# Deci-AI/super-gradients

Hardware: AMD Instinct MI355X
Metric: images/sec/node YOLO-NAS-S 640x640 train-step (higher is better)
Workload: dtype fp32 (bf16x3 MFMA); 1 GPU; YOLO-NAS-S synthetic COCO 640x640, bs=32/GPU, PPYoloELoss(TAL)+AdamW+EMA, random-init weights; global_batch=32, parallelism=dp1, conv_math=patch_bf3, conv_variant=0, bn_reduce_in_data_gradients=True, conv_tuning_entries=374, filter_planes=True

## Files before the change

### super_gradients_amd/csrc/bn.hip

```cpp
#include "sgx_common.h"
#include <atomic>

#include "sgx_sweep.h"

extern "C" int32_t sgx_stats_blocks(int64_t M) {
    long n = (M + 63) / 64;
    if (n < 1) n = 1;
    if (n > 1024) n = 1024;
    return (int32_t)n;
}

struct StatsF {
    const float* x;
    long ld;
    struct In { float4 v; };
    __device__ In load(long r, int c) const { return In{sgx_ld4(x + r * ld + c)}; }
    struct Cst {};
    __device__ Cst consts(int) const { return Cst{}; }
    __device__ void apply(long, int, const In& in, const Cst&, float4 (&q)[2]) const {
        const float4 v = in.v;
        q[0].x += v.x; q[0].y += v.y; q[0].z += v.z; q[0].w += v.w;
        q[1].x += v.x * v.x; q[1].y += v.y * v.y; q[1].z += v.z * v.z; q[1].w += v.w * v.w;
    }
};
// ... 821 lines not shown
                                          int32_t C, int32_t act, float* partials, int32_t nblk, void* stream) {
    SGX_CHECK_ARG(x1 && s1 && t1 && y, "tri_affine_act_fwd: null pointer");
    SGX_CHECK_ACT3(act, "tri_affine_act_fwd");
    SGX_CHECK_ARG(!x2 || (s2 && t2), "tri_affine_act_fwd: second branch needs scale and shift");
    SGX_CHECK_ARG(!x3 || (s3 && t3), "tri_affine_act_fwd: third branch needs scale and shift");
    SW_CHECK_VEC(C, SW_LD4(x1_ld) && (!x2 || SW_LD4(x2_ld)) && (!x3 || SW_LD4(x3_ld)) && (!r || SW_LD4(r_ld)) && SW_LD4(y_ld) && SW_ALIGNED(x1) && SW_ALIGNED(s1) && SW_ALIGNED(t1) &&
                     (!x2 || (SW_ALIGNED(x2) && SW_ALIGNED(s2) && SW_ALIGNED(t2))) && (!x3 || (SW_ALIGNED(x3) && SW_ALIGNED(s3) && SW_ALIGNED(t3))) && SW_ALIGNED(r) &&
                     SW_ALIGNED(y) && SW_ALIGNED(partials),
                 "tri_affine_act_fwd");
    Branch br[3] = {{x1, x1_ld, s1, t1, nullptr}, {x2, x2_ld, s2, t2, nullptr}, {x3, x3_ld, s3, t3, nullptr}};
    const int nb = present(br);
    const BranchSumOut o{r, r_ld, r_scale, r_scale_dev, y, y_ld};
    return nb == 1 ? branch_sum_fwd<1>(br, act, o, M, C, partials, nblk, stream)
         : nb == 2 ? branch_sum_fwd<2>(br, act, o, M, C, partials, nblk, stream)
                   : branch_sum_fwd<3>(br, act, o, M, C, partials, nblk, stream);
}

template <int NB>
struct BranchSumBwdReduceF {
    BranchSum<NB> p; const float* dy; long dy_ld; float* g; long g_ld;
    struct In { float4 x[NB], d; };
    struct Cst { typename BranchSum<NB>::Cst k; float4 m[NB]; };
    __device__ In load(long row, int c) const {
        In in;
        p.load(row, c, in.x);
        in.d = sgx_ld4(dy + row * dy_ld + c);
        return in;
    }
    __device__ Cst consts(int c) const {
        Cst k;
        k.k = p.consts(c);
#pragma unroll
        for (int i = 0; i < NB; ++i) k.m[i] = sgx_ld4(p.b[i].mean + c);
        return k;
    }
    __device__ float4 grad(const float4& d, const float4& v) const {
#pragma clang fp contract(off)
        return make_float4(d.x * sgx_act_grad(v.x, p.act), d.y * sgx_act_grad(v.y, p.act), d.z * sgx_act_grad(v.z, p.act), d.w * sgx_act_grad(v.w, p.act));
    }
    __device__ void apply(long row, int c, const In& in, const Cst& k, float4 (&q)[2 * NB]) const {
        const float4 o = grad(in.d, p.pre(k.k, in.x));
        sgx_st4(g + row * g_ld + c, o);
#pragma unroll
        for (int i = 0; i < NB; ++i) {
            const float4 e = in.x[i], m = k.m[i];
            q[2 * i].x += o.x; q[2 * i].y += o.y; q[2 * i].z += o.z; q[2 * i].w += o.w;
            q[2 * i + 1].x += o.x * (e.x - m.x); q[2 * i + 1].y += o.y * (e.y - m.y); q[2 * i + 1].z += o.z * (e.z - m.z); q[2 * i + 1].w += o.w * (e.w - m.w);
        }
    }
};
template <int NB>
static int32_t branch_sum_bwd_reduce(const Branch* br, int act, const float* dy, long dy_ld, float* g, long g_ld, long M, int C, float* partials,
                                     int nblk, void* stream) {
    return run_sweep<BranchSumBwdReduceF<NB>, 2 * NB, 2>({branch_sum<NB>(br, act), dy, dy_ld, g, g_ld}, M, C, partials, stream, "tri_affine_act_bwd_reduce", nblk);
}
extern "C" int32_t sgx_tri_affine_act_bwd_reduce(const float* dy, int64_t dy_ld, const float* x1, int64_t x1_ld, const float* s1, const float* t1,
                                                 const float* mean1, const float* x2, int64_t x2_ld, const float* s2, const float* t2,
                                                 const float* mean2, const float* x3, int64_t x3_ld, const float* s3, const float* t3,
                                                 const float* mean3, float* g, int64_t g_ld, int64_t M, int32_t C, int32_t act, float* partials,
                                                 int32_t nblk, void* stream) {
    SGX_CHECK_ARG(dy && x1 && s1 && t1 && mean1 && g && partials, "tri_affine_act_bwd_reduce: null pointer");
    SGX_CHECK_ACT3(act, "tri_affine_act_bwd_reduce");
    SGX_CHECK_ARG(!x2 || (s2 && t2 && mean2), "tri_affine_act_bwd_reduce: second branch needs scale, shift and mean");
    SGX_CHECK_ARG(!x3 || (s3 && t3 && mean3), "tri_affine_act_bwd_reduce: third branch needs scale, shift and mean");
    SW_CHECK_VEC(C, SW_LD4(dy_ld) && SW_LD4(x1_ld) && (!x2 || SW_LD4(x2_ld)) && (!x3 || SW_LD4(x3_ld)) && SW_LD4(g_ld) && SW_ALIGNED(dy) && SW_ALIGNED(x1) && SW_ALIGNED(s1) &&
                     SW_ALIGNED(t1) && SW_ALIGNED(mean1) && (!x2 || (SW_ALIGNED(x2) && SW_ALIGNED(s2) && SW_ALIGNED(t2) && SW_ALIGNED(mean2))) &&
                     (!x3 || (SW_ALIGNED(x3) && SW_ALIGNED(s3) && SW_ALIGNED(t3) && SW_ALIGNED(mean3))) && SW_ALIGNED(g) && SW_ALIGNED(partials),
                 "tri_affine_act_bwd_reduce");
    Branch br[3] = {{x1, x1_ld, s1, t1, mean1}, {x2, x2_ld, s2, t2, mean2}, {x3, x3_ld, s3, t3, mean3}};
    const int nb = present(br);
    return nb == 1 ? branch_sum_bwd_reduce<1>(br, act, dy, dy_ld, g, g_ld, M, C, partials, nblk, stream)
         : nb == 2 ? branch_sum_bwd_reduce<2>(br, act, dy, dy_ld, g, g_ld, M, C, partials, nblk, stream)
                   : branch_sum_bwd_reduce<3>(br, act, dy, dy_ld, g, g_ld, M, C, partials, nblk, stream);
}

struct ColsumF {
    const float* x; long ld; long rows_per_img; long ld_img;
    struct In { float4 v; };
    __device__ In load(long r, int c) const {
        long img = r / rows_per_img;
        return In{sgx_ld4(x + img * ld_img + (r - img * rows_per_img) * ld + c)};
    }
    struct Cst {};
    __device__ Cst consts(int) const { return Cst{}; }
    __device__ void apply(long, int, const In& in, const Cst&, float4 (&q)[1]) const {
        const float4 v = in.v;
        q[0].x += v.x; q[0].y += v.y; q[0].z += v.z; q[0].w += v.w;
    }
};
__global__ void colsum_finalize_kernel(ColSrc src, int C, float* out, int accumulate) {
    SGX_FIN_THREAD(src, C);
    double tot[1];
    col_totals<1>(src, C, c, cok, tot);
    if (!writer) return;
    const double s = tot[0];
    out[c] = accumulate ? out[c] + (float)s : (float)s;
}
extern "C" int64_t sgx_colsum_workspace(int64_t M, int32_t C) {
    int nblk = sgx_stats_blocks(M);
    return (((int64_t)nblk * C * (int64_t)sizeof(float) + 255) & ~255L) + sgx_reduce_workspace(nblk, C);
}
extern "C" int32_t sgx_colsum(const float* x, int64_t ld, int64_t M, int32_t C, int64_t rows_per_img, int64_t ld_img, float* out,
                              int32_t accumulate, float* ws, void* stream) {
    SGX_CHECK_ARG(x && out && ws && rows_per_img > 0, "colsum: bad args");
    SW_CHECK_VEC(C, SW_LD4(ld) && SW_LD4(ld_img) && SW_ALIGNED(x) && SW_ALIGNED(ws), "colsum");
    ColsumF f{x, ld, rows_per_img, ld_img};
    int32_t rc = run_sweep<ColsumF, 1, 4>(f, M, C, ws, stream, "colsum");
    if (rc) return rc;
    const int nblk = sgx_stats_blocks(M);
    const int64_t part_bytes = ((int64_t)nblk * C * (int64_t)sizeof(float) + 255) & ~255L;
    ColSrc src;
    rc = col_prereduce<1>(ws, nblk, C, (char*)ws + part_bytes, sgx_reduce_workspace(nblk, C), stream, &src);
    if (rc) return rc;
    SGX_LAUNCH(colsum_finalize_kernel, fin_grid(src, C), fin_block(src), 0, stream, src, C, out, accumulate);
    SGX_CHECK_LAUNCH("colsum_finalize");
    return SGX_OK;
}

__global__ void fill_kernel(float* p, long n, float v) {
    for (long i = (long)blockIdx.x * blockDim.x + threadIdx.x; i < n; i += (long)gridDim.x * blockDim.x) p[i] = v;
}
extern "C" int32_t sgx_fill(float* p, int64_t n, float v, void* stream) {
    if (n <= 0) return SGX_OK;
    SGX_CHECK_ARG(p, "fill: null pointer");
    long blocks = (n + 255) / 256;
    SGX_LAUNCH(fill_kernel, dim3((unsigned)(blocks > 4096 ? 4096 : blocks)), dim3(256), 0, stream, p, (long)n, v);
    SGX_CHECK_LAUNCH("fill");
    return SGX_OK;
}

__global__ void scale_dev_kernel(const float* x, const float* s, const float* t, float* y, long n) {
    float f = s[0] * (t ? t[0] : 1.f);
    for (long i = (long)blockIdx.x * blockDim.x + threadIdx.x; i < n; i += (long)gridDim.x * blockDim.x) y[i] = x[i] * f;
}
extern "C" int32_t sgx_scale_by_device_scalar(const float* x, const float* s, const float* t, float* y, int64_t n, void* stream) {
    if (n <= 0) return SGX_OK;
    SGX_CHECK_ARG(x && s && y, "scale: null pointer");
    long blocks = (n + 255) / 256;
    SGX_LAUNCH(scale_dev_kernel, dim3((unsigned)(blocks > 4096 ? 4096 : blocks)), dim3(256), 0, stream, x, s, t, y, (long)n);
    SGX_CHECK_LAUNCH("scale_by_device_scalar");
    return SGX_OK;
}

__global__ void nchw_to_nhwc_kernel(int N, int C, int H, int W, int Cpad, const float* x, float* y) {
    long n = (long)N * H * W * Cpad;
    for (long i = (long)blockIdx.x * blockDim.x + threadIdx.x; i < n; i += (long)gridDim.x * blockDim.x) {
        int c = (int)(i % Cpad);
        long pix = i / Cpad;
        long hw = (long)H * W;
        long img = pix / hw, rem = pix - img * hw;
        y[i] = c < C ? x[(img * C + c) * hw + rem] : 0.f;
    }
}
extern "C" int32_t sgx_nchw_to_nhwc(int32_t N, int32_t C, int32_t H, int32_t W, int32_t Cpad, const float* x, float* y, void* stream) {
    SGX_CHECK_ARG(x && y && Cpad >= C && Cpad % 4 == 0, "nchw_to_nhwc: bad args");
    long n = (long)N * H * W * Cpad, blocks = (n + 255) / 256;
    SGX_LAUNCH(nchw_to_nhwc_kernel, dim3((unsigned)(blocks > 8192 ? 8192 : blocks)), dim3(256), 0, stream, N, C, H, W, Cpad, x, y);
    SGX_CHECK_LAUNCH("nchw_to_nhwc");
    return SGX_OK;
}
__global__ void nhwc_to_nchw_kernel(int N, int C, int H, int W, const float* x, long ld_pix, long ld_img, float* y) {
    long n = (long)N * C * H * W;
    long hw = (long)H * W;
    for (long i = (long)blockIdx.x * blockDim.x + threadIdx.x; i < n; i += (long)gridDim.x * blockDim.x) {
        long rem = i % hw;
        long t = i / hw;
        int c = (int)(t % C);
        long img = t / C;
        y[i] = x[img * ld_img + rem * ld_pix + c];
    }
}
extern "C" int32_t sgx_nhwc_to_nchw(int32_t N, int32_t C, int32_t H, int32_t W, const float* x, int64_t x_ld_pix, int64_t x_ld_img, float* y,
                                    void* stream) {
    SGX_CHECK_ARG(x && y, "nhwc_to_nchw: null pointer");
    long n = (long)N * C * H * W, blocks = (n + 255) / 256;
    SGX_LAUNCH(nhwc_to_nchw_kernel, dim3((unsigned)(blocks > 8192 ? 8192 : blocks)), dim3(256), 0, stream, N, C, H, W, x, (long)x_ld_pix,
               (long)x_ld_img, y);
    SGX_CHECK_LAUNCH("nhwc_to_nchw");
    return SGX_OK;
}

__global__ void standardize_u8_kernel(long npix, int C, int Cpad, const uint8_t* x, float max_value, const float* mean, const float* stdv, float* y) {
    for (long i = (long)blockIdx.x * blockDim.x + threadIdx.x; i < npix; i += (long)gridDim.x * blockDim.x) {
        const uint8_t* px = x + i * C;
        float* py = y + i * Cpad;
        for (int c0 = 0; c0 < Cpad; c0 += 4) {
            float v[4];
#pragma unroll
            for (int t = 0; t < 4; ++t) {
                const int c = c0 + t;
                float f = 0.f;
                if (c < C) {
                    f = (float)px[c] / max_value;
                    if (mean) f = (f - mean[c]) / stdv[c];
                }
                v[t] = f;
            }
            sgx_st4(py + c0, make_float4(v[0], v[1], v[2], v[3]));
        }
    }
}
extern "C" int32_t sgx_standardize_u8_hwc(int32_t N, int32_t H, int32_t W, int32_t C, int32_t Cpad, const uint8_t* x, float max_value,
                                          const float* mean, const float* stdv, float* y, void* stream) {
    SGX_CHECK_ARG(x && y && N > 0 && H > 0 && W > 0 && C > 0 && Cpad >= C && Cpad % 4 == 0, "standardize_u8: bad args (C=%d Cpad=%d)", C, Cpad);
    SGX_CHECK_ARG(max_value > 0.f && ((mean == nullptr) == (stdv == nullptr)), "standardize_u8: max_value > 0, mean and std go together");
    const long npix = (long)N * H * W;
    const long blocks = (npix + 255) / 256;
    SGX_LAUNCH(standardize_u8_kernel, dim3((unsigned)(blocks > 16384 ? 16384 : blocks)), dim3(256), 0, stream, npix, C, Cpad, x, max_value, mean,
               stdv, y);
    SGX_CHECK_LAUNCH("standardize_u8");
    return SGX_OK;
}

__global__ void pad_standardize_u8_kernel(int h, int w, int C, const uint8_t* x, int H, int W, int Cpad, int top, int left, float max_value,
                                          const float* mean, const float* stdv, const float* pad_value, float* y) {
    const long npix = (long)H * W;
    for (long i = (long)blockIdx.x * blockDim.x + threadIdx.x; i < npix; i += (long)gridDim.x * blockDim.x) {
        const int yy = (int)(i / W), xx = (int)(i - (long)yy * W);
        const int sy = yy - top, sx = xx - left;
        const bool inside = sy >= 0 && sy < h && sx >= 0 && sx < w;
        const uint8_t* px = x + ((long)(inside ? sy : 0) * w + (inside ? sx : 0)) * C;
        float* py = y + i * Cpad;
        for (int c0 = 0; c0 < Cpad; c0 += 4) {
            float v[4];
#pragma unroll
            for (int t = 0; t < 4; ++t) {
                const int c = c0 + t;
                float f = 0.f;
                if (c < C) {
                    f = (inside ? (float)px[c] : pad_value[c]) / max_value;
                    if (mean) f = (f - mean[c]) / stdv[c];
                }
                v[t] = f;
            }
            sgx_st4(py + c0, make_float4(v[0], v[1], v[2], v[3]));
        }
    }
}
extern "C" int32_t sgx_pad_standardize_u8_hwc(int32_t h, int32_t w, int32_t C, const uint8_t* x, int32_t H, int32_t W, int32_t Cpad, int32_t top,
                                              int32_t left, float max_value, const float* mean, const float* stdv, const float* pad_value, float* y,
                                              void* stream) {
    SGX_CHECK_ARG(x && y && pad_value && h > 0 && w > 0 && C > 0 && Cpad >= C && Cpad % 4 == 0, "pad_standardize_u8: bad args (C=%d Cpad=%d)", C, Cpad);
    SGX_CHECK_ARG(top >= 0 && left >= 0 && top + h <= H && left + w <= W, "pad_standardize_u8: the %dx%d image at (%d, %d) does not fit %dx%d", h, w, top, left, H, W);
    SGX_CHECK_ARG(max_value > 0.f && ((mean == nullptr) == (stdv == nullptr)), "pad_standardize_u8: max_value > 0, mean and std go together");
    const long npix = (long)H * W, blocks = (npix + 255) / 256;
    SGX_LAUNCH(pad_standardize_u8_kernel, dim3((unsigned)(blocks > 8192 ? 8192 : blocks)), dim3(256), 0, stream, h, w, C, x, H, W, Cpad, top, left,
               max_value, mean, stdv, pad_value, y);
    SGX_CHECK_LAUNCH("pad_standardize_u8");
    return SGX_OK;
}

#include "dense.h"
```

### super_gradients_amd/csrc/conv.hip

```cpp
#include "sgx_common.h"

#define SGX_MAX_TAPS 64
#include <algorithm>
#include <array>
#include <atomic>
#include <map>
#include <mutex>
#include <unordered_map>
#include <vector>

#ifndef SGX_EMU
#include <mutex>
#include <vector>
namespace {
struct ProfRec {
    hipEvent_t a, b;
    double flops, bytes;
    int cls;
};
std::mutex g_prof_mu;
bool g_prof_on = false;
std::vector<ProfRec> g_prof_recs;
std::vector<hipEvent_t> g_prof_pool;
hipEvent_t prof_event() {
// ... 1817 lines not shown

extern "C" int32_t sgx_conv2d_fwd(const sgx_conv_desc* d, const float* x, const float* w, const float* bias,
                                  const float* addend, float* y, int32_t act, float* stat_partials, void* stream) {
    int32_t rc = check_desc(d);
    if (rc) return rc;
    SGX_CHECK_ARG(x && w && y, "conv fwd: null pointer");
    SGX_CHECK_ACT3(act, "conv fwd");
    TuneScope tune(0, d);
    IgemmParams p = fwd_params(d, x, w, y, stat_partials);
    p.bias = bias; p.addend = addend; p.act = act;
    return launch(plan_launch(p, 0), p, stream);
}

extern "C" int32_t sgx_conv2d_fwd_dual_stat_blocks(const sgx_conv_desc* d) {
    return plan_igemm(fwd_dual_params(d, nullptr, nullptr, nullptr, nullptr, nullptr, nullptr, nullptr), 2, true, true).mt;
}
extern "C" int32_t sgx_conv2d_fwd_dual(const sgx_conv_desc* d, const float* x, const float* w, const float* w1, const float* bias1, float* y,
                                       float* u, float* stat5, void* stream) {
    int32_t rc = check_desc(d);
    if (rc) return rc;
    SGX_CHECK_ARG(x && w && w1 && y && u && stat5, "conv fwd_dual: null pointer");
    SGX_CHECK_ARG(d->R == d->S && (d->R & 1) && d->pad == d->R / 2, "conv fwd_dual: odd square filter with pad = R / 2 (the 1x1 branch reads its centre tap)");
    SGX_CHECK_ARG(((uintptr_t)u % 16) == 0, "conv fwd_dual: needs a 16-byte aligned second output");
    SGX_CHECK_ARG(d->C >= IG_BK || d->K <= 64, "conv fwd_dual: C < 16 (the flattened K axis) has the 64-filter tiles only (K = %d)", d->K);
    IgemmParams p = fwd_dual_params(d, x, w, w1, bias1, y, u, stat5);
    return launch(plan_launch(p, 2), p, stream);
}

struct TapList {
    unsigned char idx[SGX_MAX_TAPS];
};
__global__ void wtrans_kernel(const float* w, float* wt, int K, int C, int RS, int T, TapList taps) {
    long n = (long)C * T * K;
    for (long i = (long)blockIdx.x * blockDim.x + threadIdx.x; i < n; i += (long)gridDim.x * blockDim.x) {
        int k = (int)(i % K);
        long r = i / K;
        int t = (int)(r % T);
        int c = (int)(r / T);
        wt[i] = w[((long)k * RS + taps.idx[t]) * C + c];
    }
}
__global__ void dgrad_fill_kernel(IgemmParams p) {
    const int hw = p.Ha * p.Wa;
    const long n = (long)p.M * (p.Nout / 4);
    for (long i = (long)blockIdx.x * blockDim.x + threadIdx.x; i < n; i += (long)gridDim.x * blockDim.x) {
        const int c4 = (int)(i % (p.Nout / 4)) * 4;
        const int m = (int)(i / (p.Nout / 4));
        const int img = m / hw, rem = m - img * hw, a = rem / p.Wa, b = rem - a * p.Wa;
        const long off = (long)img * p.y_ld_img + ((long)(a * p.so + p.ph) * p.Wout + (b * p.so + p.pw)) * p.y_ld_pix + c4;
        float4 v = make_float4(0.f, 0.f, 0.f, 0.f);
        if (p.bias) v = sgx_ld4(p.bias + c4);
        if (p.addend) {
            float4 u = sgx_ld4(p.addend + off);
            v.x += u.x; v.y += u.y; v.z += u.z; v.w += u.w;
        }
        if (p.accumulate) {
            float4 u = sgx_ld4(p.Y + off);
            v.x += u.x; v.y += u.y; v.z += u.z; v.w += u.w;
        }
        sgx_st4(p.Y + off, v);
    }
}

extern "C" int64_t sgx_conv2d_bwd_data_workspace(const sgx_conv_desc* d) {
    return (int64_t)d->R * d->S * d->C * d->K * sizeof(float) + 256;
}

struct DgradClass {
    int T;
    TapList taps;
    long wt_off;
    IgemmParams p;
};
#define SGX_MAX_DGRAD_CLASSES 64
static int32_t dgrad_classes(const sgx_conv_desc* d, DgradClass* cls, int* ncls) {
    int32_t rc = check_desc(d);
    if (rc) return rc;
    SGX_CHECK_ARG(d->K % 4 == 0 && d->y_ld_pix % 4 == 0, "conv bwd_data: K and dy pixel stride must be multiples of 4");
    const int s = d->stride;
    if (s > 8) SGX_FAIL(SGX_ERR_UNSUPPORTED, "conv bwd_data: stride %d (at most 8: %d output-parity classes)", s, SGX_MAX_DGRAD_CLASSES);
    int n = 0;
    long wt_off = 0;
    for (int ph = 0; ph < s; ++ph)
        for (int pw = 0; pw < s; ++pw) {
            const int Ha = (d->H - ph + s - 1) / s, Wa = (d->W - pw + s - 1) / s;
            if (Ha <= 0 || Wa <= 0) continue;
            DgradClass& c = cls[n++];
            memset(&c.taps, 0, sizeof(c.taps));
            int rows[SGX_MAX_TAPS], cols[SGX_MAX_TAPS], Th = 0, Tw = 0;
            for (int r = 0; r < d->R; ++r)
                if ((((ph + d->pad - r) % s) + s) % s == 0) rows[Th++] = r;
            for (int q = 0; q < d->S; ++q)
                if ((((pw + d->pad - q) % s) + s) % s == 0) cols[Tw++] = q;
            const int T = Th * Tw;
            for (int i = 0; i < Th; ++i)
                for (int j = 0; j < Tw; ++j) c.taps.idx[i * Tw + j] = (unsigned char)(rows[i] * d->S + cols[j]);
            c.T = T;
            c.wt_off = wt_off;
            wt_off += (long)d->C * T * d->K;
            IgemmParams& p = c.p;
            memset(&p, 0, sizeof(p));
            p.M = d->N * Ha * Wa; p.Ha = Ha; p.Wa = Wa; p.Hin = d->Ho; p.Win = d->Wo;
            p.C = d->K; p.Nout = d->C; p.Th = Th; p.Tw = Tw;
            p.dh0 = T ? (ph + d->pad - rows[0]) / s : 0;
            p.dw0 = T ? (pw + d->pad - cols[0]) / s : 0;
            p.dstep = -1;
            p.si = 1; p.so = s; p.ph = ph; p.pw = pw; p.Hout = d->H; p.Wout = d->W;
            p.a_ld_pix = d->y_ld_pix; p.a_ld_img = d->y_ld_img; p.y_ld_pix = d->x_ld_pix; p.y_ld_img = d->x_ld_img;
            p.w_ld_n = (long)T * d->K;
            p.a_bytes = view_bytes(d->N, d->Ho, d->Wo, d->K, d->y_ld_pix, d->y_ld_img);
            p.w_bytes = (long)d->C * p.w_ld_n * 4;
            p.act = SGX_ACT_NONE;
        }
    *ncls = n;
    return SGX_OK;
}
struct DgradSecond {
    const float* ds;
    long ld_pix, ld_img;
    const float* w1t;
    const float* addend2;
    long a2_ld_pix, a2_ld_img;
    float a2_scale;
    const float* a2_scale_dev;
};
static void dgrad_second(IgemmParams& p, const sgx_conv_desc* d, const DgradSecond* sec) {
    p.Hin2 = d->Ho; p.Win2 = d->Wo; p.Th2 = 1; p.Tw2 = 1; p.dh02 = 0; p.dw02 = 0; p.dstep2 = 1;
    p.w2_ld_n = d->K;
    p.w2_bytes = (long)d->C * d->K * 4;
    if (!sec) return;
    p.A2 = sec->ds; p.Wt2 = sec->w1t;
    p.a2_ld_pix = sec->ld_pix; p.a2_ld_img = sec->ld_img;
    p.a2_bytes = view_bytes(d->N, d->Ho, d->Wo, d->K, sec->ld_pix, sec->ld_img);
    p.addend2 = sec->addend2; p.a2d_ld_pix = sec->a2_ld_pix; p.a2d_ld_img = sec->a2_ld_img;
    p.addend2_scale = sec->a2_scale; p.addend2_scale_dev = sec->a2_scale_dev;
}

extern "C" int32_t sgx_conv2d_transpose_weights(const sgx_conv_desc* d, const float* w, float* wt, int64_t wt_bytes, void* stream) {
    DgradClass cls[SGX_MAX_DGRAD_CLASSES];
    int n = 0;
    int32_t rc = dgrad_classes(d, cls, &n);
    if (rc) return rc;
    SGX_CHECK_ARG(w, "conv bwd_data: null pointer");
    if (wt_bytes < sgx_conv2d_bwd_data_workspace(d) || !wt) SGX_FAIL(SGX_ERR_WORKSPACE, "conv bwd_data: workspace too small");
    for (int i = 0; i < n; ++i) {
        if (!cls[i].T) continue;
        const long e = (long)d->C * cls[i].T * d->K;
        const int grid = (int)((e + 255) / 256 > 2048 ? 2048 : (e + 255) / 256);
        SGX_LAUNCH(wtrans_kernel, dim3(grid), dim3(256), 0, stream, w, wt + cls[i].wt_off, d->K, d->C, d->R * d->S, cls[i].T, cls[i].taps);
        SGX_CHECK_LAUNCH("wtrans");
    }
    return SGX_OK;
}
__global__ void wtrans_batch_kernel(const sgx_wtrans_job* jobs) {
    __shared__ sgx_wtrans_job job;
    if (threadIdx.x == 0) job = jobs[blockIdx.y];
    __syncthreads();
    const unsigned n = (unsigned)job.C * (unsigned)job.T * (unsigned)job.K, K = (unsigned)job.K, T = (unsigned)job.T;
    for (unsigned i = blockIdx.x * blockDim.x + threadIdx.x; i < n; i += gridDim.x * blockDim.x) {
        const unsigned k = i % K, r = i / K, t = r % T, c = r / T;
        job.wt[i] = job.w[((long)k * job.RS + job.taps[t]) * job.C + c];
    }
}
extern "C" int32_t sgx_wtrans_batch(const sgx_wtrans_job* jobs_dev, int32_t njobs, void* stream) {
    SGX_CHECK_ARG(jobs_dev && njobs > 0 && njobs <= 65535, "wtrans_batch: bad args (njobs=%d)", njobs);
    SGX_LAUNCH(wtrans_batch_kernel, dim3(SGX_STRIDE_GRID(256), (unsigned)njobs), dim3(256), 0, stream, jobs_dev);
    SGX_CHECK_LAUNCH("wtrans_batch");
    return SGX_OK;
}
__global__ void qarep_prep_kernel(const sgx_qarep_prep_job* jobs) {
    __shared__ sgx_qarep_prep_job job;
    if (threadIdx.x == 0) job = jobs[blockIdx.y];
    __syncthreads();
    const long n = (long)job.K * job.C;
    const float a = job.alpha ? job.alpha[0] : 1.f;
    for (long i = (long)blockIdx.x * blockDim.x + threadIdx.x; i < n; i += (long)gridDim.x * blockDim.x) {
        const int c = (int)(i % job.C), k = (int)(i / job.C);
        const float v = a * job.w1[i] + ((job.identity && k == c) ? 1.f : 0.f);
        job.w1p[i] = v;
        job.w1pt[(long)c * job.K + k] = v;
    }
}
extern "C" int32_t sgx_qarep_prep_batch(const sgx_qarep_prep_job* jobs_dev, int32_t njobs, void* stream) {
    SGX_CHECK_ARG(jobs_dev && njobs > 0 && njobs <= 65535, "qarep_prep_batch: bad args (njobs=%d)", njobs);
    SGX_LAUNCH(qarep_prep_kernel, dim3(SGX_STRIDE_GRID(8), (unsigned)njobs), dim3(256), 0, stream, jobs_dev);
    SGX_CHECK_LAUNCH("qarep_prep_batch");
    return SGX_OK;
}
extern "C" int32_t sgx_conv2d_transpose_jobs(const sgx_conv_desc* d, const float* w, float* wt, int64_t wt_bytes, sgx_wtrans_job* jobs,
                                             int32_t max_jobs, int32_t* njobs) {
    SGX_CHECK_ARG(jobs && njobs && max_jobs > 0, "transpose_jobs: null pointer");
    DgradClass cls[SGX_MAX_DGRAD_CLASSES];
    int n = 0;
    int32_t rc = dgrad_classes(d, cls, &n);
    if (rc) return rc;
    SGX_CHECK_ARG(w, "conv bwd_data: null pointer");
    if (wt_bytes < sgx_conv2d_bwd_data_workspace(d) || !wt) SGX_FAIL(SGX_ERR_WORKSPACE, "conv bwd_data: workspace too small");
    int nj = 0;
    for (int i = 0; i < n; ++i) {
        if (!cls[i].T) continue;
        if (nj < max_jobs) {
            sgx_wtrans_job& j = jobs[nj];
            memset(&j, 0, sizeof(j));
            j.w = w; j.wt = wt + cls[i].wt_off; j.K = d->K; j.C = d->C; j.RS = d->R * d->S; j.T = cls[i].T;
            memcpy(j.taps, cls[i].taps.idx, sizeof(cls[i].taps.idx) < sizeof(j.taps) ? sizeof(cls[i].taps.idx) : sizeof(j.taps));
        }
        ++nj;
    }
    if (nj > max_jobs) SGX_FAIL(SGX_ERR_BAD_ARG, "transpose_jobs: %d jobs, room for %d", nj, max_jobs);
    *njobs = nj;
    return SGX_OK;
}

extern "C" int32_t sgx_conv2d_bwd_data_stat_blocks(const sgx_conv_desc* d, int32_t two_source) {
    DgradClass cls[SGX_MAX_DGRAD_CLASSES];
    int n = 0, rows = 0;
    if (dgrad_classes(d, cls, &n)) return 0;
    TuneScope tune(1, d);
    for (int i = 0; i < n; ++i) {
        if (!cls[i].T) return 0;
        const int ph2 = two_source && cls[i].p.ph == 0 && cls[i].p.pw == 0;
        if (ph2) dgrad_second(cls[i].p, d, nullptr);
        const ConvPlan pl = plan_igemm(cls[i].p, ph2, true, false);
        if (pl.err || !pl.req_ok) return 0;
        rows += pl.mt;
    }
    return rows;
}

static int32_t dgrad_launch(const sgx_conv_desc* d, const float* dy, const float* wt, const float* bias, const float* addend, float* dx,
                            int32_t accumulate, const DgradSecond* sec, const sgx_bn_reduce_req* reqs, int nreq, void* stream) {
    DgradClass cls[SGX_MAX_DGRAD_CLASSES];
    ConvPlan plans[SGX_MAX_DGRAD_CLASSES];
    int n = 0, rows = 0;
    int32_t rc = dgrad_classes(d, cls, &n);
    if (rc) return rc;
    SGX_CHECK_ARG(dy && dx, "conv bwd_data: null pointer");
    if (!wt) SGX_FAIL(SGX_ERR_WORKSPACE, "conv bwd_data: workspace too small");
    SGX_CHECK_ARG(nreq >= 0 && nreq <= SGX_MAX_BN_REQ && (nreq == 0 || reqs), "conv bwd_data: bad BatchNorm-reduce requests");
    for (int r = 0; r < nreq; ++r)
        SGX_CHECK_ARG(reqs[r].t && reqs[r].scale && reqs[r].shift && reqs[r].mean && reqs[r].partials && reqs[r].c_lo >= 0 && reqs[r].c_hi <= d->C &&
                          reqs[r].c_lo < reqs[r].c_hi && reqs[r].c_lo % 4 == 0 && reqs[r].c_hi % 4 == 0 && reqs[r].t_ld_pix % 4 == 0 &&
                          reqs[r].t_ld_img % 4 == 0 && ((uintptr_t)reqs[r].t % 16) == 0 && ((uintptr_t)reqs[r].scale % 16) == 0 &&
                          ((uintptr_t)reqs[r].shift % 16) == 0 && ((uintptr_t)reqs[r].mean % 16) == 0,
                      "conv bwd_data: BatchNorm-reduce request %d: null pointer, unaligned operand or a channel range outside [0, C)", r);
    for (int r = 0; r < nreq; ++r) SGX_CHECK_ACT3(reqs[r].act, "conv bwd_data: BatchNorm-reduce request");
    TuneScope tune(1, d);
    for (int i = 0; i < n; ++i) {
        IgemmParams& p = cls[i].p;
        p.A = dy; p.Wt = wt + cls[i].wt_off; p.bias = bias; p.addend = addend; p.Y = dx; p.accumulate = accumulate;
        const int ph2 = sec && p.ph == 0 && p.pw == 0;
        if (ph2) dgrad_second(p, d, sec);
        if (cls[i].T) {
            plans[i] = plan_launch(p, ph2);
            if (plans[i].err) SGX_FAIL(plans[i].err, "%s", plans[i].msg);
        }
        if (!nreq) continue;
        if (!cls[i].T || !plans[i].req_ok)
            SGX_FAIL(SGX_ERR_UNSUPPORTED, "conv bwd_data: this problem cannot carry BatchNorm-reduce requests (sgx_conv2d_bwd_data_stat_blocks = 0)");
        p.nreq = nreq;
        p.req_row0 = rows;
        rows += plans[i].mt;
        for (int r = 0; r < nreq; ++r) {
            p.req[r].t = reqs[r].t; p.req[r].scale = reqs[r].scale; p.req[r].shift = reqs[r].shift; p.req[r].mean = reqs[r].mean;
            p.req[r].parts = reqs[r].partials; p.req[r].t_ld_pix = reqs[r].t_ld_pix; p.req[r].t_ld_img = reqs[r].t_ld_img;
            p.req[r].c_lo = reqs[r].c_lo; p.req[r].c_hi = reqs[r].c_hi; p.req[r].act = reqs[r].act; p.req[r].rows = reqs[r].rows;
        }
    }
    for (int r = 0; r < nreq; ++r)
        SGX_CHECK_ARG(reqs[r].rows == rows, "conv bwd_data: request %d was allocated for %d rows, the launch writes %d (sgx_conv2d_bwd_data_stat_blocks)", r, reqs[r].rows, rows);
    for (int i = 0; i < n; ++i) {
        IgemmParams& p = cls[i].p;
        if (cls[i].T) {
            rc = launch(plans[i], p, stream);
            if (rc) return rc;
        } else if (!(accumulate && !addend && !bias)) {
            const long e = (long)p.M * (p.Nout / 4);
            const int grid = (int)((e + 255) / 256 > 4096 ? 4096 : (e + 255) / 256);
            SGX_LAUNCH(dgrad_fill_kernel, dim3(grid), dim3(256), 0, stream, p);
            SGX_CHECK_LAUNCH("dgrad_fill");
        }
    }
    return SGX_OK;
}
extern "C" int32_t sgx_conv2d_bwd_data(const sgx_conv_desc* d, const float* dy, const float* w, const float* addend,
                                       float* dx, int32_t accumulate, void* ws, int64_t ws_bytes, void* stream) {
    SGX_CHECK_ARG(dy && dx, "conv bwd_data: null pointer");
    int32_t rc = sgx_conv2d_transpose_weights(d, w, (float*)ws, ws_bytes, stream);
    return rc ? rc : dgrad_launch(d, dy, (const float*)ws, nullptr, addend, dx, accumulate, nullptr, nullptr, 0, stream);
}
extern "C" int32_t sgx_conv2d_bwd_data_wt(const sgx_conv_desc* d, const float* dy, const float* wt, const float* addend, float* dx,
                                          int32_t accumulate, void* stream) {
    return dgrad_launch(d, dy, wt, nullptr, addend, dx, accumulate, nullptr, nullptr, 0, stream);
}
extern "C" int32_t sgx_conv2d_bwd_data_wt_req(const sgx_conv_desc* d, const float* dy, const float* wt, const float* addend, float* dx,
                                              int32_t accumulate, const sgx_bn_reduce_req* reqs, int32_t nreq, void* stream) {
    return dgrad_launch(d, dy, wt, nullptr, addend, dx, accumulate, nullptr, reqs, nreq, stream);
}
extern "C" int32_t sgx_conv2d_bwd_data_dual_req(const sgx_conv_desc* d, const float* dy, const float* wt, const float* ds, int64_t ds_ld_pix,
                                                int64_t ds_ld_img, const float* w1t, const float* addend, const float* addend2, int64_t a2_ld_pix,
                                                int64_t a2_ld_img, float a2_scale, const float* a2_scale_dev, float* dx, int32_t accumulate,
                                                const sgx_bn_reduce_req* reqs, int32_t nreq, void* stream) {
    SGX_CHECK_ARG(ds && w1t && d && d->K >= IG_BK && ds_ld_pix % 4 == 0, "conv bwd_data_dual: bad args (needs K >= 16)");
    SGX_CHECK_ARG(!addend2 || (d->stride == 1 && a2_ld_pix % 4 == 0 && a2_ld_img % 4 == 0 && ((uintptr_t)addend2 % 16) == 0),
                  "conv bwd_data_dual: the scaled second addend needs stride 1 and 16-byte aligned rows");
    DgradSecond sec{ds, (long)ds_ld_pix, (long)ds_ld_img, w1t, addend2, (long)a2_ld_pix, (long)a2_ld_img, a2_scale, a2_scale_dev};
    return dgrad_launch(d, dy, wt, nullptr, addend, dx, accumulate, &sec, reqs, nreq, stream);
}
extern "C" int32_t sgx_conv2d_bwd_data_dual(const sgx_conv_desc* d, const float* dy, const float* wt, const float* ds, int64_t ds_ld_pix,
                                            int64_t ds_ld_img, const float* w1t, const float* addend, const float* addend2, int64_t a2_ld_pix,
                                            int64_t a2_ld_img, float a2_scale, const float* a2_scale_dev, float* dx, int32_t accumulate,
                                            void* stream) {
    return sgx_conv2d_bwd_data_dual_req(d, dy, wt, ds, ds_ld_pix, ds_ld_img, w1t, addend, addend2, a2_ld_pix, a2_ld_img, a2_scale, a2_scale_dev, dx,
                                        accumulate, nullptr, 0, stream);
}

#define WG_BKP 16
#define WG_BKP_DEEP 32
#define WG_MAX_SPLIT 4096
#define WG_MAX_JOBS 24

struct WgJob {
    const float* X;
    const float* DY;
    float* dw;
    float* part;
    int* tickets;
    long x_ld_pix, x_ld_img, y_ld_pix, y_ld_img;
    long x_bytes, dy_bytes;
    int H, W, C, K, S, stride, pad, Ho, Wo;
    int M, J, ksplit, mchunk, kt_tiles, jt_tiles;
    int blk0;
};
struct WgGroupParams {
    int njobs, xcd_order;
    WgFold fold;
    int blk0[WG_MAX_JOBS];
    WgJob jobs[WG_MAX_JOBS];
};

constexpr int wg_min_waves(int acc_regs, int pf) { return acc_regs <= 16 ? 1 : (acc_regs == 32 && pf == 2) ? 4 : 512 / (acc_regs + (pf == 2 ? 64 : 48)); }
constexpr int wg_bf16_pitch(int row) { return row + (row % 64 == 0 ? 32 : 0); }
template <int BNK, int BJ, int WK, int WC, int BKP, int PF, int MATH = 0>
__global__ __launch_bounds__(WK * WC * 64, MATH ? 1 : wg_min_waves((BNK / (WK * 32)) * (BJ / (WC * 32)) * 16, PF)) void wgrad_kernel(WgGroupParams g) {
    constexpr int NTH = WK * WC * 64;
    constexpr int TK = BNK / (WK * 32), TC = BJ / (WC * 32);
    static_assert(TK >= 1 && TC >= 1 && TK * WK * 32 == BNK && TC * WC * 32 == BJ, "bad tile");
    static_assert(MATH == 0 || BKP == 16, "bf16x3 loop: 16-pixel slabs (one K step of the bf16 MFMA)");
    constexpr int G = NTH / BKP;
    constexpr int DJ = (BNK / 4 + G - 1) / G, XJ = (BJ / 4 + G - 1) / G;
    constexpr int DP = wg_bf16_pitch(BNK), XP = wg_bf16_pitch(BJ);
    __shared__ float Ds[MATH ? 4 : 2 * BKP * BNK];
    __shared__ float Xs[MATH ? 4 : 2 * BKP * BJ];
    __shared__ unsigned short Dh[MATH ? 2 * 3 * BKP * DP : 4];
    __shared__ unsigned short Xh[MATH ? 2 * 3 * BKP * XP : 4];
    __shared__ int s_last;

    const int tid = threadIdx.x, lane = tid & 63, wave = tid >> 6;
// ... 730 lines not shown
```

### super_gradients_amd/csrc/loss.hip

```cpp
#include "sgx_common.h"

#define LOSS_THREADS 256
#define TAL_EPS 1e-9f

struct LossWs {
    float* pbox;
    int* cnt;
    int* sel;
    int* agt;
    float* am;
    float* aiou;
    unsigned* maxm;
    unsigned* maxi;
    float* partials;
    long bytes;
};

static long align_up(long v) { return (v + 255) & ~255L; }

static LossWs carve(const sgx_loss_desc* d, void* ws) {
    LossWs w;
    char* p = (char*)ws;
    long BL = (long)d->B * d->L, Bn = (long)d->B * (d->nmax > 0 ? d->nmax : 1);
    long off = 0;
// ... 46 lines not shown
        float v = -1.f;
        if (t < T) v = targets[(long)t * 6];
        const bool hit = t < T && (int)v == b && v == (float)b;
        const unsigned long long bits = __ballot(hit);
        if (hit) {
            const int slot = n + __popcll(bits & ((1ull << lane) - 1ull));
            if (slot < nmax) gt_index[(long)b * nmax + slot] = t;
        }
        n += __popcll(bits);
    }
    if (lane == 0) {
        gt_count[b] = n < nmax ? n : nmax;
        if (n > nmax) atomicAdd(overflow, n - nmax);
    }
    for (int i = n + lane; i < nmax; i += 64) gt_index[(long)b * nmax + i] = -1;
}
extern "C" int32_t sgx_targets_index(const float* targets, int32_t T, int32_t B, int32_t nmax, int32_t* gt_count, int32_t* gt_index,
                                     int32_t* overflow, void* stream) {
    SGX_CHECK_ARG(gt_count && overflow && B > 0 && T >= 0 && nmax >= 0, "targets_index: bad args");
    SGX_CHECK_ARG(T == 0 || targets, "targets_index: null targets");
    SGX_CHECK_ARG(nmax == 0 || gt_index, "targets_index: null gt_index");
    SGX_MEMSET_ASYNC(overflow, 0, sizeof(int), stream);
    SGX_LAUNCH(targets_index_kernel, dim3(B), dim3(64), 0, stream, targets, T, B, nmax, gt_count, gt_index, overflow);
    SGX_CHECK_LAUNCH("targets_index");
    return SGX_OK;
}

__device__ __forceinline__ void softmax_expect(const float* d, int R1, float& e) {
    float m = d[0];
    for (int j = 1; j < R1; ++j) m = fmaxf(m, d[j]);
    float s = 0.f, acc = 0.f;
    for (int j = 0; j < R1; ++j) {
        float ex = expf(d[j] - m);
        s += ex;
        acc += ex * (float)j;
    }
    e = acc / s;
}
#define DEC_MAXR1 33
template <bool PX>
__global__ __launch_bounds__(256) void decode_rows_kernel(int B, int L, int R1, const float* distri, const float* points, const float* strides, float mul_stride,
                                                          float* boxes) {
    __shared__ float rows[256 * DEC_MAXR1];
    const long n = (long)B * L * 4;
    for (long i0 = (long)blockIdx.x * 256; i0 < n; i0 += (long)gridDim.x * 256) {
        const long cnt = (n - i0 < 256 ? n - i0 : 256) * R1;
        const float* src = distri + i0 * R1;
        for (long q = threadIdx.x; q < cnt; q += 256) rows[q] = src[q];
        __syncthreads();
        const long i = i0 + threadIdx.x;
        if (i < n) {
            const int k = (int)(i & 3);
            const int l = (int)((i >> 2) % L);
            float e;
            softmax_expect(rows + threadIdx.x * R1, R1, e);
            if (PX) {
                const float pc = points[2 * l + (k & 1)] / strides[l];
                boxes[i] = k < 2 ? pc - e : pc + e;
            } else {
                const float pc = points[2 * l + (k & 1)];
                const float sc = mul_stride != 0.f ? strides[l] : 1.f;
                boxes[i] = (k < 2 ? pc - e : pc + e) * sc;
            }
        }
        __syncthreads();
    }
}
__global__ void decode_kernel(int B, int L, int R1, const float* distri, const float* points_grid, const float* strides, float mul_stride,
                              float* boxes) {
    long n = (long)B * L * 4;
    for (long i = (long)blockIdx.x * blockDim.x + threadIdx.x; i < n; i += (long)gridDim.x * blockDim.x) {
        const int k = (int)(i & 3);
        const int l = (int)((i >> 2) % L);
        float e;
        softmax_expect(distri + i * R1, R1, e);
        const float pc = points_grid[2 * l + (k & 1)];
        const float s = mul_stride != 0.f ? strides[l] : 1.f;
        boxes[i] = (k < 2 ? pc - e : pc + e) * s;
    }
}
__global__ void sigmoid_kernel(const float* x, float* y, long n) {
    for (long i = (long)blockIdx.x * blockDim.x + threadIdx.x; i < n; i += (long)gridDim.x * blockDim.x) y[i] = sigmoidf(x[i]);
}
extern "C" int32_t sgx_dfl_decode(int32_t B, int32_t L, int32_t C, int32_t reg_max, const float* logits, const float* distri,
                                  const float* points_grid, const float* strides, float* boxes, float* scores, void* stream) {
    SGX_CHECK_ARG(distri && points_grid && strides && boxes, "dfl_decode: null pointer");
    long n = (long)B * L, blocks = (4 * n + 255) / 256;
    if (reg_max + 1 <= DEC_MAXR1)
        SGX_LAUNCH(decode_rows_kernel<false>, dim3((unsigned)(blocks > 16384 ? 16384 : blocks)), dim3(256), 0, stream, B, L, reg_max + 1, distri, points_grid,
                   strides, 1.f, boxes);
    else
        SGX_LAUNCH(decode_kernel, dim3((unsigned)(blocks > 16384 ? 16384 : blocks)), dim3(256), 0, stream, B, L, reg_max + 1, distri, points_grid,
                   strides, 1.f, boxes);
    SGX_CHECK_LAUNCH("dfl_decode");
    if (scores) {
        SGX_CHECK_ARG(logits, "dfl_decode: scores requested without logits");
        long m = n * C, b2 = (m + 255) / 256;
        SGX_LAUNCH(sigmoid_kernel, dim3((unsigned)(b2 > 8192 ? 8192 : b2)), dim3(256), 0, stream, logits, scores, m);
        SGX_CHECK_LAUNCH("sigmoid");
    }
    return SGX_OK;
}

__device__ __forceinline__ void block_argbest(float v, int idx, bool want_max, float* sv, int* si, float& out_v, int& out_i) {
    for (int off = 32; off > 0; off >>= 1) {
        float ov = __shfl_down(v, off);
        int oi = __shfl_down(idx, off);
        bool better = want_max ? (ov > v || (ov == v && oi < idx)) : (ov < v || (ov == v && oi < idx));
        if (oi >= 0 && (idx < 0 || better)) {
            v = ov;
            idx = oi;
        }
    }
    const int wave = threadIdx.x >> 6, lane = threadIdx.x & 63;
    if (lane == 0) {
        sv[wave] = v;
        si[wave] = idx;
    }
    __syncthreads();
    if (threadIdx.x == 0) {
        float bv = sv[0];
        int bi = si[0];
        for (int w = 1; w < (int)(blockDim.x >> 6); ++w) {
            float ov = sv[w];
            int oi = si[w];
            bool better = want_max ? (ov > bv || (ov == bv && oi < bi)) : (ov < bv || (ov == bv && oi < bi));
            if (oi >= 0 && (bi < 0 || better)) {
                bv = ov;
                bi = oi;
            }
        }
        sv[0] = bv;
        si[0] = bi;
    }
    __syncthreads();
    out_v = sv[0];
    out_i = si[0];
    __syncthreads();
}

__global__ __launch_bounds__(LOSS_THREADS) void tal_candidates_kernel(sgx_loss_desc d, const float* logits, const float* points,
                                                                      const float* strides, const float* targets, const int* gt_count,
                                                                      const int* gt_index, LossWs w, int topk, float alpha, float beta) {
    SGX_DYN_SMEM(float, metric);
    __shared__ float sv[LOSS_THREADS / 64];
    __shared__ int si[LOSS_THREADS / 64];
    const int g = blockIdx.x, b = blockIdx.y;
    if (g >= gt_count[b]) return;
    const float* t = targets + (long)gt_index[(long)b * d.nmax + g] * 6;
    const Box gt = target_box(t);
    const int cls = (int)t[1];
    bool valid = (gt.x1 + gt.y1 + gt.x2 + gt.y2) > 0.f;
    const int L = d.L;
    for (int l = threadIdx.x; l < L; l += LOSS_THREADS) {
        const float* pb = w.pbox + ((long)b * L + l) * 4;
        const float s = strides[l];
        Box p{pb[0] * s, pb[1] * s, pb[2] * s, pb[3] * s};
        float iou = pair_iou(gt, p, 1e-9f);
        float sc = sigmoidf(logits[((long)b * L + l) * d.C + cls]);
        float m = powf(sc, alpha) * powf(iou, beta);
        bool in = point_in_box(points[2 * l], points[2 * l + 1], gt);
        metric[l] = in ? m : 0.f;
    }
    __syncthreads();
    const int k = topk < L ? topk : L;
    for (int round = 0; round < k; ++round) {
        float bv = -1.f;
        int bi = -1;
        for (int l = threadIdx.x; l < L; l += LOSS_THREADS) {
            float v = metric[l];
            if (v > bv) {
                bv = v;
                bi = l;
            }
        }
        float rv;
        int ri;
        block_argbest(bv, bi, true, sv, si, rv, ri);
        if (ri < 0) break;
        if (round == 0 && d.sequential_assignment) valid = rv > 1e-9f;
        if (threadIdx.x == 0) {
            metric[ri] = -2.f;
            if (valid && point_in_box(points[2 * ri], points[2 * ri + 1], gt)) {
                atomicAdd(&w.cnt[(long)b * L + ri], 1);
                w.sel[(long)b * L + ri] = g;
            }
        }
        __syncthreads();
    }
}

#define ATSS_MAXCAND 128
__global__ __launch_bounds__(LOSS_THREADS) void atss_candidates_kernel(sgx_loss_desc d, const float* anchors, const float* targets,
                                                                       const int* gt_count, const int* gt_index, LossWs w, int topk) {
    SGX_DYN_SMEM(float, dist);
    __shared__ float sv[LOSS_THREADS / 64];
    __shared__ int si[LOSS_THREADS / 64];
    __shared__ int cand[ATSS_MAXCAND];
    __shared__ float ciou[ATSS_MAXCAND];
    const int g = blockIdx.x, b = blockIdx.y;
    if (g >= gt_count[b]) return;
    const float* t = targets + (long)gt_index[(long)b * d.nmax + g] * 6;
    const Box gt = target_box(t);
    const bool valid = d.sequential_assignment ? true : (gt.x1 + gt.y1 + gt.x2 + gt.y2) > 0.f;
    const int L = d.L;
    const float gcx = (gt.x1 + gt.x2) / 2.f, gcy = (gt.y1 + gt.y2) / 2.f;
    for (int l = threadIdx.x; l < L; l += LOSS_THREADS) {
        const float* a = anchors + (long)l * 4;
        float acx = (a[0] + a[2]) / 2.f, acy = (a[1] + a[3]) / 2.f;
        float dx = gcx - acx, dy = gcy - acy;
        dist[l] = sqrtf(dx * dx + dy * dy);
    }
    __syncthreads();
    int ncand = 0, off = 0;
    for (int lev = 0; lev < d.num_levels; ++lev) {
        const int n = d.level_count[lev];
        const int k = topk < n ? topk : n;
        for (int round = 0; round < k; ++round) {
            float bv = 3.0e38f;
            int bi = -1;
            for (int l = off + (int)threadIdx.x; l < off + n; l += LOSS_THREADS) {
                float v = dist[l];
                if (v < bv) {
                    bv = v;
                    bi = l;
                }
            }
            float rv;
            int ri;
            block_argbest(bv, bi, false, sv, si, rv, ri);
            if (ri < 0) break;
            if (threadIdx.x == 0) {
                dist[ri] = 3.3e38f;
                if (ncand + round < ATSS_MAXCAND) cand[ncand + round] = ri;
            }
            __syncthreads();
        }
        ncand += k;
        off += n;
    }
    if (ncand > ATSS_MAXCAND) ncand = ATSS_MAXCAND;
    for (int i = threadIdx.x; i < ncand; i += LOSS_THREADS) {
        const float* a = anchors + (long)cand[i] * 4;
        Box ab{a[0], a[1], a[2], a[3]};
        ciou[i] = valid ? pair_iou(gt, ab, 1e-10f) : 0.f;
    }
    __syncthreads();
    if (threadIdx.x == 0) {
        float mean = 0.f;
        for (int i = 0; i < ncand; ++i) mean += ciou[i];
        mean /= (float)ncand;
        float var = 0.f;
        for (int i = 0; i < ncand; ++i) var += (ciou[i] - mean) * (ciou[i] - mean);
        float sd = ncand > 1 ? sqrtf(var / (float)(ncand - 1)) : 0.f;
        float thr = mean + sd;
        for (int i = 0; i < ncand; ++i) {
            int l = cand[i];
            const float* a = anchors + (long)l * 4;
            float acx = (a[0] + a[2]) / 2.f, acy = (a[1] + a[3]) / 2.f;
            if (valid && ciou[i] > thr && point_in_box(acx, acy, gt)) {
                atomicAdd(&w.cnt[(long)b * L + l], 1);
                w.sel[(long)b * L + l] = g;
            }
        }
    }
}

__global__ void resolve_kernel(sgx_loss_desc d, const float* logits, const float* anchors, const float* strides, const float* targets,
                               const int* gt_count, const int* gt_index, LossWs w, float alpha, float beta) {
    long n = (long)d.B * d.L;
    for (long i = (long)blockIdx.x * blockDim.x + threadIdx.x; i < n; i += (long)gridDim.x * blockDim.x) {
        const int b = (int)(i / d.L), l = (int)(i % d.L);
        const int c = w.cnt[i];
        int g = -1;
        const float s = strides[l];
        const float* pb = w.pbox + i * 4;
        Box p{pb[0] * s, pb[1] * s, pb[2] * s, pb[3] * s};
        if (c == 1) g = w.sel[i];
        else if (c > 1) {
            float best = -1.f;
            Box q = p;
            if (d.use_static_assigner) {
                const float* a = anchors + (long)l * 4;
                q = Box{a[0], a[1], a[2], a[3]};
            }
            const int ng = gt_count[b];
            for (int k = 0; k < ng; ++k) {
                Box gt = target_box(targets + (long)gt_index[(long)b * d.nmax + k] * 6);
                float v = pair_iou(gt, q, d.use_static_assigner ? 1e-10f : 1e-9f);
                if (v > best) {
                    best = v;
                    g = k;
                }
            }
        }
        w.agt[i] = g;
        float m = 0.f, iou = 0.f;
        if (g >= 0) {
            const float* t = targets + (long)gt_index[(long)b * d.nmax + g] * 6;
            Box gt = target_box(t);
            iou = pair_iou(gt, p, 1e-9f);
            if (!d.use_static_assigner) {
                float sc = sigmoidf(logits[i * d.C + (int)t[1]]);
                m = powf(sc, alpha) * powf(iou, beta);
                atomicMax((int*)&w.maxm[(long)b * d.nmax + g], __float_as_int(m));
                atomicMax((int*)&w.maxi[(long)b * d.nmax + g], __float_as_int(iou));
            }
        }
        w.am[i] = m;
        w.aiou[i] = iou;
    }
}

__global__ __launch_bounds__(LOSS_THREADS) void box_loss_kernel(sgx_loss_desc d, const float* distri, const float* points, const float* strides,
                                                                const float* targets, const int* gt_index, LossWs w, int* assigned_label,
                                                                float* assigned_box, float* assigned_score, float* g_distri, float* partials) {
    __shared__ float red[3][LOSS_THREADS];
    const int R1 = d.reg_max + 1;
    const long n = (long)d.B * d.L;
    const long i = (long)blockIdx.x * LOSS_THREADS + threadIdx.x;
    float l_iou = 0.f, l_dfl = 0.f, s_sum = 0.f;
    if (i < n) {
        const int b = (int)(i / d.L), l = (int)(i % d.L);
        const int g = w.agt[i];
        float* gd = g_distri + i * 4 * R1;
        if (g < 0) {
            assigned_label[i] = d.C;
            float bx[4] = {0.f, 0.f, 0.f, 0.f};
            if (d.nmax > 0 && gt_index[(long)b * d.nmax] >= 0) {
                Box g0 = target_box(targets + (long)gt_index[(long)b * d.nmax] * 6);
                bx[0] = g0.x1; bx[1] = g0.y1; bx[2] = g0.x2; bx[3] = g0.y2;
            }
            for (int k = 0; k < 4; ++k) assigned_box[i * 4 + k] = bx[k];
            assigned_score[i] = 0.f;
            for (int k = 0; k < 4 * R1; ++k) gd[k] = 0.f;
        } else {
            const float* t = targets + (long)gt_index[(long)b * d.nmax + g] * 6;
            const Box gt = target_box(t);
            float score;
            if (d.use_static_assigner) score = w.aiou[i];
            else {
// ... 358 lines not shown
```

Before: 781.1 images/s.

## Tile weight transposes, vectorize 4-channel NHWC pack, incremental TAL top-k scan

New measurement: 783.4 images/s (median of 6 runs). No clear change (+0.3%).

```diff
diff --git a/super_gradients_amd/csrc/bn.hip b/super_gradients_amd/csrc/bn.hip
--- a/super_gradients_amd/csrc/bn.hip
+++ b/super_gradients_amd/csrc/bn.hip
@@ -997,8 +997,40 @@
         y[i] = c < C ? x[(img * C + c) * hw + rem] : 0.f;
     }
 }
+#define NHWC4_Q 2
+__global__ __launch_bounds__(256) void nchw_to_nhwc4_kernel(int C, unsigned hwq, unsigned nq, const float* x, float* y) {
+    const unsigned step = gridDim.x * blockDim.x;
+    for (unsigned q0 = blockIdx.x * blockDim.x + threadIdx.x; q0 < nq; q0 += NHWC4_Q * step) {
+        float4 p[NHWC4_Q][4];
+#pragma unroll
+        for (int u = 0; u < NHWC4_Q; ++u) {
+            const unsigned q = q0 + u * step;
+            const unsigned img = q / hwq, rq = q - img * hwq;
+            const float* const xp = x + ((size_t)img * C * hwq + rq) * 4;
+#pragma unroll
+            for (int c = 0; c < 4; ++c) p[u][c] = (q < nq && c < C) ? sgx_ld4(xp + (size_t)c * hwq * 4) : make_float4(0.f, 0.f, 0.f, 0.f);
+        }
+#pragma unroll
+        for (int u = 0; u < NHWC4_Q; ++u) {
+            const unsigned q = q0 + u * step;
+            if (q >= nq) break;
+            float* const yp = y + (size_t)q * 16;
+            sgx_st4(yp, make_float4(p[u][0].x, p[u][1].x, p[u][2].x, p[u][3].x));
+            sgx_st4(yp + 4, make_float4(p[u][0].y, p[u][1].y, p[u][2].y, p[u][3].y));
+            sgx_st4(yp + 8, make_float4(p[u][0].z, p[u][1].z, p[u][2].z, p[u][3].z));
+            sgx_st4(yp + 12, make_float4(p[u][0].w, p[u][1].w, p[u][2].w, p[u][3].w));
+        }
+    }
+}
 extern "C" int32_t sgx_nchw_to_nhwc(int32_t N, int32_t C, int32_t H, int32_t W, int32_t Cpad, const float* x, float* y, void* stream) {
     SGX_CHECK_ARG(x && y && Cpad >= C && Cpad % 4 == 0, "nchw_to_nhwc: bad args");
+    const long hw = (long)H * W, quads = (long)N * hw / 4;
+    if (Cpad == 4 && C > 0 && hw % 4 == 0 && quads > 0 && quads < (1L << 30) && ((uintptr_t)x % 16) == 0 && ((uintptr_t)y % 16) == 0) {
+        const long wg = (quads + 256 * NHWC4_Q - 1) / (256 * NHWC4_Q);
+        SGX_LAUNCH(nchw_to_nhwc4_kernel, dim3((unsigned)(wg > 8192 ? 8192 : wg)), dim3(256), 0, stream, C, (unsigned)(hw / 4), (unsigned)quads, x, y);
+        SGX_CHECK_LAUNCH("nchw_to_nhwc4");
+        return SGX_OK;
+    }
     long n = (long)N * H * W * Cpad, blocks = (n + 255) / 256;
     SGX_LAUNCH(nchw_to_nhwc_kernel, dim3((unsigned)(blocks > 8192 ? 8192 : blocks)), dim3(256), 0, stream, N, C, H, W, Cpad, x, y);
     SGX_CHECK_LAUNCH("nchw_to_nhwc");
diff --git a/super_gradients_amd/csrc/conv.hip b/super_gradients_amd/csrc/conv.hip
--- a/super_gradients_amd/csrc/conv.hip
+++ b/super_gradients_amd/csrc/conv.hip
@@ -1993,38 +1993,73 @@
     }
     return SGX_OK;
 }
-__global__ void wtrans_batch_kernel(const sgx_wtrans_job* jobs) {
+#define TR_TILE 32
+#define TR_ROWS (256 / TR_TILE)
+static inline int tr_tiles(int K, int C) { return sgx_cdiv(K, TR_TILE) * sgx_cdiv(C, TR_TILE); }
+static std::atomic<int> g_wt_max_tiles{1};
+#define TR_MAX_GRID 512
+__global__ __launch_bounds__(256) void wtrans_batch_kernel(const sgx_wtrans_job* jobs) {
     __shared__ sgx_wtrans_job job;
+    __shared__ float tile[TR_TILE][TR_TILE + 1];
+    const unsigned K = (unsigned)jobs[blockIdx.y].K, C = (unsigned)jobs[blockIdx.y].C, T = (unsigned)jobs[blockIdx.y].T;
+    const unsigned kt = (K + TR_TILE - 1) / TR_TILE, ct = (C + TR_TILE - 1) / TR_TILE, ntiles = T * kt * ct;
+    if (blockIdx.x >= ntiles) return;
     if (threadIdx.x == 0) job = jobs[blockIdx.y];
     __syncthreads();
-    const unsigned n = (unsigned)job.C * (unsigned)job.T * (unsigned)job.K, K = (unsigned)job.K, T = (unsigned)job.T;
-    for (unsigned i = blockIdx.x * blockDim.x + threadIdx.x; i < n; i += gridDim.x * blockDim.x) {
-        const unsigned k = i % K, r = i / K, t = r % T, c = r / T;
-        job.wt[i] = job.w[((long)k * job.RS + job.taps[t]) * job.C + c];
+    const unsigned tx = threadIdx.x % TR_TILE, ty = threadIdx.x / TR_TILE;
+    for (unsigned i = blockIdx.x; i < ntiles; i += gridDim.x) {
+        const unsigned c0 = (i % ct) * TR_TILE, r = i / ct, k0 = (r % kt) * TR_TILE, t = r / kt;
+        const float* const src = job.w + (size_t)job.taps[t] * C;
+#pragma unroll
+        for (unsigned j = ty; j < TR_TILE; j += TR_ROWS)
+            if (k0 + j < K && c0 + tx < C) tile[j][tx] = src[(size_t)(k0 + j) * job.RS * C + c0 + tx];
+        __syncthreads();
+#pragma unroll
+        for (unsigned j = ty; j < TR_TILE; j += TR_ROWS)
+            if (c0 + j < C && k0 + tx < K) job.wt[((size_t)(c0 + j) * T + t) * K + k0 + tx] = tile[tx][j];
+        __syncthreads();
     }
 }
 extern "C" int32_t sgx_wtrans_batch(const sgx_wtrans_job* jobs_dev, int32_t njobs, void* stream) {
     SGX_CHECK_ARG(jobs_dev && njobs > 0 && njobs <= 65535, "wtrans_batch: bad args (njobs=%d)", njobs);
-    SGX_LAUNCH(wtrans_batch_kernel, dim3(SGX_STRIDE_GRID(256), (unsigned)njobs), dim3(256), 0, stream, jobs_dev);
+    const int gx = std::min(TR_MAX_GRID, g_wt_max_tiles.load());
+    SGX_LAUNCH(wtrans_batch_kernel, dim3(SGX_STRIDE_GRID(gx), (unsigned)njobs), dim3(256), 0, stream, jobs_dev);
     SGX_CHECK_LAUNCH("wtrans_batch");
     return SGX_OK;
 }
-__global__ void qarep_prep_kernel(const sgx_qarep_prep_job* jobs) {
+#define QAREP_GRID 256
+__global__ __launch_bounds__(256) void qarep_prep_kernel(const sgx_qarep_prep_job* jobs) {
     __shared__ sgx_qarep_prep_job job;
+    __shared__ float tile[TR_TILE][TR_TILE + 1];
+    const unsigned K = (unsigned)jobs[blockIdx.y].K, C = (unsigned)jobs[blockIdx.y].C;
+    const unsigned ct = (C + TR_TILE - 1) / TR_TILE, ntiles = ((K + TR_TILE - 1) / TR_TILE) * ct;
+    const unsigned tx = threadIdx.x % TR_TILE, ty = threadIdx.x / TR_TILE;
+    if (blockIdx.x >= ntiles) return;
     if (threadIdx.x == 0) job = jobs[blockIdx.y];
     __syncthreads();
-    const long n = (long)job.K * job.C;
     const float a = job.alpha ? job.alpha[0] : 1.f;
-    for (long i = (long)blockIdx.x * blockDim.x + threadIdx.x; i < n; i += (long)gridDim.x * blockDim.x) {
-        const int c = (int)(i % job.C), k = (int)(i / job.C);
-        const float v = a * job.w1[i] + ((job.identity && k == c) ? 1.f : 0.f);
-        job.w1p[i] = v;
-        job.w1pt[(long)c * job.K + k] = v;
+    for (unsigned t = blockIdx.x; t < ntiles; t += gridDim.x) {
+        const unsigned c0 = (t % ct) * TR_TILE, k0 = (t / ct) * TR_TILE;
+#pragma unroll
+        for (unsigned j = ty; j < TR_TILE; j += TR_ROWS) {
+            const unsigned k = k0 + j, c = c0 + tx;
+            if (k < K && c < C) {
+                const size_t i = (size_t)k * C + c;
+                const float v = a * job.w1[i] + ((job.identity && k == c) ? 1.f : 0.f);
+                job.w1p[i] = v;
+                tile[j][tx] = v;
+            }
+        }
+        __syncthreads();
+#pragma unroll
+        for (unsigned j = ty; j < TR_TILE; j += TR_ROWS)
+            if (c0 + j < C && k0 + tx < K) job.w1pt[(size_t)(c0 + j) * K + k0 + tx] = tile[tx][j];
+        __syncthreads();
     }
 }
 extern "C" int32_t sgx_qarep_prep_batch(const sgx_qarep_prep_job* jobs_dev, int32_t njobs, void* stream) {
     SGX_CHECK_ARG(jobs_dev && njobs > 0 && njobs <= 65535, "qarep_prep_batch: bad args (njobs=%d)", njobs);
-    SGX_LAUNCH(qarep_prep_kernel, dim3(SGX_STRIDE_GRID(8), (unsigned)njobs), dim3(256), 0, stream, jobs_dev);
+    SGX_LAUNCH(qarep_prep_kernel, dim3(SGX_STRIDE_GRID(QAREP_GRID), (unsigned)njobs), dim3(256), 0, stream, jobs_dev);
     SGX_CHECK_LAUNCH("qarep_prep_batch");
     return SGX_OK;
 }
@@ -2045,6 +2080,9 @@
             memset(&j, 0, sizeof(j));
             j.w = w; j.wt = wt + cls[i].wt_off; j.K = d->K; j.C = d->C; j.RS = d->R * d->S; j.T = cls[i].T;
             memcpy(j.taps, cls[i].taps.idx, sizeof(cls[i].taps.idx) < sizeof(j.taps) ? sizeof(cls[i].taps.idx) : sizeof(j.taps));
+            const int tiles = (int)std::min((long)TR_MAX_GRID, (long)cls[i].T * tr_tiles(d->K, d->C));
+            int seen = g_wt_max_tiles.load();
+            while (tiles > seen && !g_wt_max_tiles.compare_exchange_weak(seen, tiles)) {}
         }
         ++nj;
     }
diff --git a/super_gradients_amd/csrc/loss.hip b/super_gradients_amd/csrc/loss.hip
--- a/super_gradients_amd/csrc/loss.hip
+++ b/super_gradients_amd/csrc/loss.hip
@@ -222,21 +222,37 @@
     const int cls = (int)t[1];
     bool valid = (gt.x1 + gt.y1 + gt.x2 + gt.y2) > 0.f;
     const int L = d.L;
-    for (int l = threadIdx.x; l < L; l += LOSS_THREADS) {
-        const float* pb = w.pbox + ((long)b * L + l) * 4;
-        const float s = strides[l];
-        Box p{pb[0] * s, pb[1] * s, pb[2] * s, pb[3] * s};
-        float iou = pair_iou(gt, p, 1e-9f);
-        float sc = sigmoidf(logits[((long)b * L + l) * d.C + cls]);
-        float m = powf(sc, alpha) * powf(iou, beta);
-        bool in = point_in_box(points[2 * l], points[2 * l + 1], gt);
-        metric[l] = in ? m : 0.f;
-    }
-    __syncthreads();
+    constexpr int TAL_PTS = 4;
+    for (int l0 = threadIdx.x; l0 < L; l0 += TAL_PTS * LOSS_THREADS) {
+        float px[TAL_PTS], py[TAL_PTS];
+#pragma unroll
+        for (int u = 0; u < TAL_PTS; ++u) {
+            const int l = l0 + u * LOSS_THREADS;
+            px[u] = l < L ? points[2 * l] : 0.f;
+            py[u] = l < L ? points[2 * l + 1] : 0.f;
+        }
+#pragma unroll
+        for (int u = 0; u < TAL_PTS; ++u) {
+            const int l = l0 + u * LOSS_THREADS;
+            if (l >= L) break;
+            float m = 0.f;
+            if (point_in_box(px[u], py[u], gt)) {
+                const float* pb = w.pbox + ((long)b * L + l) * 4;
+                const float s = strides[l];
+                Box p{pb[0] * s, pb[1] * s, pb[2] * s, pb[3] * s};
+                float iou = pair_iou(gt, p, 1e-9f);
+                float sc = sigmoidf(logits[((long)b * L + l) * d.C + cls]);
+                m = powf(sc, alpha) * powf(iou, beta);
+            }
+            metric[l] = m;
+        }
+    }
     const int k = topk < L ? topk : L;
-    for (int round = 0; round < k; ++round) {
-        float bv = -1.f;
-        int bi = -1;
+    float bv;
+    int bi;
+    auto scan_own = [&]() {
+        bv = -1.f;
+        bi = -1;
         for (int l = threadIdx.x; l < L; l += LOSS_THREADS) {
             float v = metric[l];
             if (v > bv) {
@@ -244,19 +260,24 @@
                 bi = l;
             }
         }
+    };
+    scan_own();
+    for (int round = 0; round < k; ++round) {
         float rv;
         int ri;
         block_argbest(bv, bi, true, sv, si, rv, ri);
         if (ri < 0) break;
         if (round == 0 && d.sequential_assignment) valid = rv > 1e-9f;
         if (threadIdx.x == 0) {
-            metric[ri] = -2.f;
             if (valid && point_in_box(points[2 * ri], points[2 * ri + 1], gt)) {
                 atomicAdd(&w.cnt[(long)b * L + ri], 1);
                 w.sel[(long)b * L + ri] = g;
             }
         }
-        __syncthreads();
+        if (ri % LOSS_THREADS == (int)threadIdx.x) {
+            metric[ri] = -2.f;
+            scan_own();
+        }
     }
 }
 
```
